# cremebrule/rgb-proprioceptive-pose-estimator

Measured on AMD Instinct MI355X. Metric: images/sec (train step, 224x224 bs256 per GPU), higher is better.
Workload: dtype bf16

## Files before the change

include/rpe_hip.h:

```cpp
#ifndef RPE_HIP_H
#define RPE_HIP_H

#ifdef __cplusplus
extern "C" {
#endif

#define RPE_ABI_VERSION 3

enum { RPE_F32 = 0, RPE_BF16 = 1, RPE_F16 = 2 };
enum {
    RPE_OK = 0,
    RPE_ERR_SHAPE = 1,
    RPE_ERR_DTYPE = 2,
    RPE_ERR_ALIGN = 3,
    RPE_ERR_HIP = 4,
    RPE_ERR_WORKSPACE = 5,
    RPE_ERR_STATE = 6
};

int rpe_abi_version(void);
const char* rpe_build_id(void);
const char* rpe_last_error(void);

typedef struct {
// ... 336 lines not shown
int rpe_resnet50_aux_head_bwd(rpe_resnet50_t* e, const float* dout, long ld_dout, const float* w, const float* depth_feat, const float* raw,
                              const unsigned char* idx, float* dw, float* dbias, float* d_depth_feat, float* workspace, long workspace_floats, void* stream);
int rpe_resnet50_forward(rpe_resnet50_t* e, const float* img_nchw, float* features, long ld_features, int training, void* stream);
int rpe_resnet50_forward_u8(rpe_resnet50_t* e, const unsigned char* frames, int Hs, int Ws, const float* mean3_host, const float* std3_host,
                            float* features, long ld_features, int training, void* stream);
typedef struct {
    int Hr, Wr, top, left, ksx, ksy;
    const int *xb, *xk, *yb, *yk;
    unsigned char* tmp;
} rpe_resize_plan;
int rpe_resnet50_forward_u8_resized(rpe_resnet50_t* e, const unsigned char* frames, int Hs, int Ws, const rpe_resize_plan* rs, const float* mean3_host,
                                    const float* std3_host, float* features, long ld_features, int training, void* stream);
const void* rpe_resnet50_early_feature(const rpe_resnet50_t* e);
void* rpe_resnet50_early_grad(rpe_resnet50_t* e);
int rpe_resnet50_backward(rpe_resnet50_t* e, const float* d_features, long ld_d_features, int use_d_early, void* stream);
enum { RPE_PROF_CONV_FWD = 0, RPE_PROF_CONV_DGRAD = 1, RPE_PROF_CONV_WGRAD = 2, RPE_PROF_BN_FWD = 3, RPE_PROF_BN_BWD = 4,
       RPE_PROF_OTHER = 5, RPE_PROF_NUM = 6 };
int rpe_resnet50_profile(rpe_resnet50_t* e, int enable);
int rpe_resnet50_profile_read(rpe_resnet50_t* e, float* ms, int* launches, double* flops, double* bytes);
long rpe_resnet50_profile_kernels(rpe_resnet50_t* e, char* buf, long buflen);
const char* rpe_last_kernel_name(void);
void rpe_set_walk_direction(int mode);
int rpe_conv2d_wgrad_halo_min_width(int width);
int rpe_resnet50_backward_begin(rpe_resnet50_t* e, const float* d_features, long ld_d_features, void* stream);
int rpe_resnet50_backward_blocks(rpe_resnet50_t* e, int count, int join, void* stream);
int rpe_resnet50_backward_end(rpe_resnet50_t* e, int use_d_early, void* stream);
int rpe_resnet50_backward_frozen(rpe_resnet50_t* e, const float* d_features, long ld_d_features, void* stream);
int rpe_resnet50_set_aux_grad(rpe_resnet50_t* e, const float* aux_dout, long aux_ld, const float* aux_depth_feat, const unsigned char* aux_idx,
                              const float* aux_w);
int rpe_resnet50_tensor(const rpe_resnet50_t* e, const char* name, const void** ptr, long* rows, int* channels);
int rpe_resnet50_set_hook_grad(rpe_resnet50_t* e, int layer, const void* dense_grad);
int rpe_resnet50_set_stem_raw(rpe_resnet50_t* e, int on);

#ifdef __cplusplus
}
#endif
#endif
```

rgb-proprioceptive-pose-estimator_amd/_lib.py:

```python
import ctypes
import os

import torch
from ctypes import POINTER, Structure, c_char_p, c_double, c_float, c_int, c_long, c_void_p

_HERE = os.path.dirname(os.path.abspath(__file__))
LIB_PATH = os.environ.get("RPE_LIB_PATH") or os.path.join(_HERE, "librpe_hip.so")

RPE_F32, RPE_BF16, RPE_F16 = 0, 1, 2
ABI_VERSION = 3
PARAM_STATS_COLS, PARAM_STATS_PART_COLS = 10, 8


class RpeError(RuntimeError):
    """A librpe_hip.so entry point returned a non-zero status."""


class BnBwdEpilogue(Structure):
    _fields_ = [(n, c_void_p) for n in ("y", "a_out", "mean", "invstd", "scale", "shift", "stats_part", "a_mask")]


class ResizePlan(Structure):
    _fields_ = [(n, c_int) for n in ("Hr", "Wr", "top", "left", "ksx", "ksy")] + [(n, c_void_p) for n in ("xb", "xk", "yb", "yk", "tmp")]

# ... 8 lines not shown


class AugmentDesc(Structure):
    _fields_ = ([("seed", ctypes.c_ulonglong)] + [(n, c_int) for n in ("qb_lo", "qb_hi", "qc_lo", "qc_hi", "qs_lo", "qs_hi", "noise_q")]
                + [("erase_thresh", ctypes.c_uint)] + [(n, c_int) for n in ("eh_lo", "eh_hi", "ew_lo", "ew_hi", "fill_mode")]
                + [("fill_rgb", ctypes.c_ubyte * 3), ("group", c_int)])


class SampleDesc(Structure):
    _fields_ = [("seed", ctypes.c_ulonglong)] + [(n, c_int) for n in ("E", "T", "S", "stride", "N", "shuffle")]


class MeasureDesc(Structure):
    _fields_ = [("seed", ctypes.c_ulonglong)] + [(n, c_int) for n in ("S", "N", "num_scales")] + [("sigma", c_double * 8), ("rho", c_double)]


class DropoutDesc(Structure):
    _fields_ = [("seed", ctypes.c_ulonglong), ("thresh", ctypes.c_uint), ("scale", c_float)]


class DepthAugmentDesc(Structure):
    _fields_ = ([("seed", ctypes.c_ulonglong)] + [(n, c_double) for n in ("n0", "n1", "n2", "q", "inv_q", "lo", "hi")] + [("drop_thresh", ctypes.c_uint)]
                + [(n, c_int) for n in ("hole_lo", "hole_hi", "hh_lo", "hh_hi", "hw_lo", "hw_hi")] + [("hole_value", c_float), ("occluder_value", c_float),
                                                                                                       ("group", c_int)])


class OcclusionDesc(Structure):
    _fields_ = [(n, c_int) for n in ("Hs", "Ws", "ph", "pw", "sy", "sx")] + [("fill_rgb", ctypes.c_ubyte * 3)]


class OverlayStyle(Structure):
    _fields_ = [("rgb", ctypes.c_ubyte * 3), ("axis_rgb", ctypes.c_ubyte * 9)] + [(n, c_int) for n in ("alpha_q8", "r_q4", "hw_q4", "trail", "trail_r_q4")]


OVERLAY_INVALID, OVERLAY_NEAR, OVERLAY_CLAMP_Q4, OVERLAY_AXIS_Q4 = -2 ** 31, 2.0 ** -10, 2 ** 17, 2 ** 13
OVERLAY_MAX_SETS, OVERLAY_MAX_TRAIL, OVERLAY_MAX_RADIUS_Q4, OVERLAY_MAX_SIDE = 4, 64, 256, 4096

P, I, L, F, D = c_void_p, c_int, c_long, c_float, c_double
PD = POINTER(ConvDesc)

_SPEC = {
    "rpe_abi_version": (I, []),
    "rpe_last_error": (c_char_p, []),
    "rpe_build_id": (c_char_p, []),
    "rpe_x4_bytes": (L, [I, I, I, I]),
    "rpe_conv_out_hw": (I, [PD, POINTER(c_int), POINTER(c_int)]),
    "rpe_conv_stats_tiles": (L, [L]),
    "rpe_conv2d_fwd": (I, [PD, I, P, P, P, P, P]),
    "rpe_conv2d_fwd_affine": (I, [PD, I, P, P, P, P, P, I, P]),
    "rpe_conv2d_fwd_affine_workspace_bytes": (L, [PD, I]),
    "rpe_conv2d_fwd_affine_ws": (I, [PD, I, P, P, P, P, P, I, P, L, P]),
    "rpe_conv2d_dgrad": (I, [PD, I, P, P, P, P, P]),
    "rpe_conv2d_dgrad_stats_tiles": (L, [PD, I]),
    "rpe_conv2d_fwd_stats_tiles": (L, [PD, I]),
    "rpe_conv2d_dgrad_bn": (I, [PD, I, P, P, P, P, POINTER(BnBwdEpilogue), P]),
    "rpe_conv1x1s2_dgrad_compact": (I, [PD, I, P, P, P, P]),
    "rpe_conv2d_dgrad_sub": (I, [PD, I, P, P, P, P, P]),
    "rpe_conv2d_dgrad_bn_sub": (I, [PD, I, P, P, P, P, POINTER(BnBwdEpilogue), P]),
    "rpe_conv1x1_dgrad_kcat_y_sub": (I, [PD, I, P, P, P, P, P, P, POINTER(BnBwdEpilogue), P]),
    "rpe_bn_backward_reduce": (I, [I, P, P, P, P, P, P, P, P, L, I, P, L, P, P, P]),
    "rpe_bn_backward_from_dz": (I, [I, P, P, P, P, P, P, I, P, P, P, L, I, P, P, P]),
    "rpe_bn_bwd_fold_scratch_bytes": (L, [I, I, I]),
    "rpe_bn_bwd_fold_conv1x1": (I, [I, I, I, P, P, P, P, P, P, P, P, P, L, P]),
    "rpe_conv1x1_dgrad_kcat": (I, [PD, I, P, P, P, P, P, POINTER(BnBwdEpilogue), P]),
    "rpe_bn_bwd_fold_y_conv1x1": (I, [I, I, I, P, P, P, P, P, P, P, P]),
    "rpe_conv1x1_dgrad_kcat_y": (I, [PD, I, P, P, P, P, P, P, POINTER(BnBwdEpilogue), P]),
# ... 105 lines not shown
    "rpe_resnet50_profile": (I, [P, I]),
    "rpe_resnet50_profile_read": (I, [P, POINTER(c_float), POINTER(c_int), POINTER(c_double), POINTER(c_double)]),
    "rpe_resnet50_backward_begin": (I, [P, P, L, P]),
    "rpe_resnet50_backward_blocks": (I, [P, I, I, P]),
    "rpe_resnet50_backward_end": (I, [P, I, P]),
    "rpe_resnet50_backward_frozen": (I, [P, P, L, P]),
    "rpe_resnet50_set_aux_grad": (I, [P, P, L, P, P, P]),
    "rpe_resnet50_profile_kernels": (L, [P, P, L]),
    "rpe_last_kernel_name": (c_char_p, []),
    "rpe_set_walk_direction": (None, [I]),
    "rpe_conv2d_wgrad_halo_min_width": (I, [I]),
    "rpe_resnet50_set_aux_head": (I, [P, P, P, P, P, L, P, P]),
    "rpe_resnet50_aux_head_bwd": (I, [P, P, L, P, P, P, P, P, P, P, P, L, P]),
    "rpe_aux_head_bwd_det_y": (I, [I, P, L, P, P, P, P, P, P, P, P, P, P, I, I, I, P, L, P]),
    "rpe_bn_apply_maxpool3x3s2_aux": (I, [I, P, P, P, P, P, P, I, I, I, P, P, P, P, L, P, P, P]),
    "rpe_resnet50_side_stream_info": (I, [P, POINTER(c_int), POINTER(c_int)]),
    "rpe_resnet50_tensor": (I, [P, c_char_p, POINTER(c_void_p), POINTER(c_long), POINTER(c_int)]),
    "rpe_resnet50_set_hook_grad": (I, [P, I, P]),
    "rpe_resnet50_set_stem_raw": (I, [P, I]),
    "rpe_aux_head_fwd_c": (I, [I, P, I, P, P, P, P, L, P, P, I, I, I, P]),
    "rpe_aux_head_bwd_c": (I, [I, P, L, P, I, P, P, P, P, P, P, P, P, I, I, I, P]),
    "rpe_depth_head_fwd_pools": (I, [P, P, P, P, P, I, I, I, I, P]),
    "rpe_tensor_add": (I, [I, P, P, L, P]),
    "rpe_feature_planes": (I, [I, P, I, I, I, I, P, P, P]),
    "rpe_feature_planes_batch": (I, [I, P, I, I, I, I, P, P, P]),
    "rpe_feature_mosaic": (I, [P, P, I, I, I, I, I, I, P, P]),
    "rpe_occlusion_grid": (L, [POINTER(OcclusionDesc), POINTER(c_int), POINTER(c_int)]),
    "rpe_occlude_grid_u8": (I, [P, P, I, I, POINTER(OcclusionDesc), P]),
    "rpe_pose_displacement": (I, [P, P, L, P, P, P]),
    "rpe_saliency_map": (I, [P, I, POINTER(OcclusionDesc), P, P, P]),
    "rpe_saliency_overlay_u8": (I, [P, P, P, P, I, I, I, I, P, P]),
    "rpe_project_poses": (I, [P, P, P, L, I, I, D, P, P, D, D, I, P, P, P]),
    "rpe_draw_poses_u8": (I, [P, P, L, I, I, P, P, L, I, POINTER(OverlayStyle), I, I, POINTER(ctypes.c_ubyte), I, P]),
}
_NOT_STATUS = {"rpe_abi_version", "rpe_conv2d_wgrad_halo_min_width", "rpe_grad_sumsq_rows", "rpe_param_stats_rows"}

EXPORTS = tuple(_SPEC)


def _load():
    if not os.path.exists(LIB_PATH):
        raise ImportError(
            "librpe_hip.so not found at %s -- build it with `python __graft_entry__.py build` "
            "(hipcc --offload-arch=gfx950); there is no fallback path." % LIB_PATH
        )
    lib = ctypes.CDLL(LIB_PATH)
    for name, (res, args) in _SPEC.items():
        try:
            fn = getattr(lib, name)
        except AttributeError as e:
            raise ImportError("librpe_hip.so does not export %s (stale build?)" % name) from e
        fn.restype = res
        fn.argtypes = args
    if lib.rpe_abi_version() != ABI_VERSION:
        raise ImportError("librpe_hip.so ABI version %d != expected %d" % (lib.rpe_abi_version(), ABI_VERSION))
    return lib


_raw = _load()


class _Checked:

    def __getattr__(self, name):
        fn = getattr(_raw, name)
        res = _SPEC[name][0]
# ... 17 lines not shown
```

rgb-proprioceptive-pose-estimator_amd/headops.py:

```python
import os

import torch

from . import ops
from ._lib import lib

pad4 = ops.pad4


def new_rows(rows, cols, device, zero=True):
    buf = (torch.zeros if zero else torch.empty)((rows, pad4(cols)), dtype=torch.float32, device=device)
    return buf[:, :cols]


def _grad_of(p):
    g = getattr(p, "_rpe_grad", None)
    if g is None:
        raise RuntimeError("parameter has no arena gradient view (model not materialised on the device)")
    return g


class LinearOp:

    def __init__(self, weight, bias, relu=False):
# ... 27 lines not shown
            self.x, self.y = x, out
        return out

    def bwd(self, dy, need_dx=True, accumulate=False):
        n, k = self.weight.shape
        x, y = self.x, self.y
        m = x.shape[0]
        if self.relu:
            if y.stride(0) != pad4(n) or dy.stride(0) != pad4(n):
                raise RuntimeError("LinearOp.bwd: ReLU layers need [M, pad4(N)] row buffers")
            ypad = y.as_strided((m, pad4(n)), (pad4(n), 1), y.storage_offset())
            dypad = dy.as_strided((m, pad4(n)), (pad4(n), 1), dy.storage_offset())
            dy = ops.relu_bwd(ypad, dypad)[:, :n]
        gw = _grad_of(self.weight)
        if k % 4 == 0 and gw.is_contiguous():
            ops.linear_wgrad(dy, x, gw, n=n, k=k, overwrite=not accumulate)
        else:
            tmp = torch.zeros((n, pad4(k)), dtype=torch.float32, device=dy.device)
            ops.linear_wgrad(dy, x, tmp, n=n, k=pad4(k))
            if accumulate:
                gw.add_(tmp[:, :k])
            else:
                ops.copy2d(tmp, gw, cols=k)
        if self.bias is not None:
            ops.colsum(dy, cols=n, out=_grad_of(self.bias), accumulate=accumulate)
        if not need_dx:
            return None
        wt = ops.transpose_f32(self.weight.data, ldo=pad4(n))
        dx = new_rows(m, k, dy.device)
        ops.linear_fwd(dy, wt, None, relu=False, out=dx, n=k, k=pad4(n))
        return dx


class LSTMOp:

    def __init__(self, w_ih, w_hh, b_ih, b_hh):
        self.w_ih, self.w_hh, self.b_ih, self.b_hh = w_ih, w_hh, b_ih, b_hh
        self.in_lin = LinearOp(w_ih, None, relu=False)
        self.hidden = w_hh.shape[1]
        if self.hidden % 4:
            raise ValueError("LSTM hidden size must be a multiple of 4 (16-byte rows)")

    def fwd(self, x, S, N, h0=None, c0=None, save=True):
        H = self.hidden
        dev = x.device
        xg = self.in_lin.fwd(x, save=save)
        gates = torch.empty((S, N, 4 * H), dtype=torch.float32, device=dev)
        hs = torch.empty((S, N, H), dtype=torch.float32, device=dev)
        cs = torch.empty((S, N, H), dtype=torch.float32, device=dev)
        whh = self.w_hh.data
        s = ops._stream()
        for t in range(S):
            h_prev = h0 if t == 0 else hs[t - 1]
            c_prev = c0 if t == 0 else cs[t - 1]
            xg_t = xg[t * N:(t + 1) * N]
            if h_prev is None:
                gates[t].copy_(xg_t)
            else:
                ops.linear_fwd(h_prev, whh, None, addend=xg_t, out=gates[t], n=4 * H, k=H)
            lib.rpe_lstm_cell_fwd(ops._p(gates[t]), ops._p(self.b_ih.data), ops._p(self.b_hh.data), ops._p(c_prev), ops._p(cs[t]), ops._p(hs[t]),
                                  N, H, s)
        if save:
            if h0 is not None:
                h0 = h0.clone()
            if c0 is not None:
                c0 = c0.clone()
# ... 200 lines not shown
```

rgb-proprioceptive-pose-estimator_amd/models/naive.py:

```python
import torch
import torch.nn as nn

from .. import ops
from ..headops import LinearOp, new_rows
from ._core import PoseModelBase, Replicated


class NaiveEndEffectorStateEstimator(PoseModelBase):

    def __init__(self, hidden_dims_pre_measurement, hidden_dims_post_measurement, num_resnet_layers=50, latent_dim=50,
                 feature_extract=True, compute_dtype=None):
        super().__init__()
        self._init_features(num_resnet_layers, latent_dim, feature_extract, True, None, False, wrap=False, register_heads=True,
                            compute_dtype=compute_dtype)
        pre = [latent_dim] + list(hidden_dims_pre_measurement) + [7]
        for i in range(len(pre) - 1):
            setattr(self, "pre_fc{}".format(i), nn.Linear(pre[i], pre[i + 1]))
        self.n_pre_hidden = len(pre) - 1
        post = [latent_dim + 7] + list(hidden_dims_post_measurement) + [7]
        for i in range(len(post) - 1):
            setattr(self, "post_fc{}".format(i), nn.Linear(post[i], post[i + 1]))
        self.n_post_hidden = len(post) - 1
        self._pre_ops = [LinearOp(getattr(self, "pre_fc%d" % i).weight, getattr(self, "pre_fc%d" % i).bias, relu=True)
                         for i in range(self.n_pre_hidden)]
        self._post_ops = [LinearOp(getattr(self, "post_fc%d" % i).weight, getattr(self, "post_fc%d" % i).bias, relu=True)
                          for i in range(self.n_post_hidden)]

    def forward(self, img, depth, self_measurement):
        return self._call(img, depth, self_measurement)

    def _flat_inputs(self, img, depth, x0bar):
        return (img.shape[0],), img, None, x0bar

    def _feature_rows(self, img, depth, save):
        feat = new_rows(img.shape[0], self.latent_dim, img.device)
        self._features_fwd(img, None, feat, save)
        return feat

    def _heads_fwd(self, feat, lead, x0bar, save):
        n, L = feat.shape[0], self.latent_dim
        h = feat
        for op in self._pre_ops:
            h = op.fwd(h, save=save)
        pre = h
        post_in = new_rows(n, L + 7, feat.device)
        ops.copy2d(feat, post_in, cols=L)
        ops.copy2d((pre - x0bar).contiguous(), post_in[:, L:], cols=7)
        h = post_in
        for op in self._post_ops:
            h = op.fwd(h, save=save)
        return pre.contiguous(), h.contiguous()

    def _backward_impl(self, d_outs):
        L = self.latent_dim
        d_pre, d_post = d_outs
        dev = self._pre_ops[0].x.device
        n = self._pre_ops[0].x.shape[0]
        d = self._pad_rows(d_post, 7) if d_post is not None else new_rows(n, 7, dev)
        for op in reversed(self._post_ops):
            d = op.bwd(d)
        d_feat = new_rows(n, L, dev)
        ops.copy2d(d, d_feat, cols=L)
        d_pre_total = d[:, L:L + 7].contiguous()
        if d_pre is not None:
            d_pre_total = d_pre_total + d_pre.reshape(n, 7)
        d = self._pad_rows(d_pre_total, 7)
        for op in reversed(self._pre_ops):
            d = op.bwd(d)
        d_feat.add_(d)
        self._features_bwd(d_feat)

    def reset_initial_state(self, batch_size):
        pass

    @property
    def requires_sequence(self):
        return False


class NaiveObjectStateEstimator(PoseModelBase):

    def __init__(self, object_name, hidden_dims, num_resnet_layers=50, latent_dim=50, feature_extract=True,
                 feature_layer_nums=(9,), use_depth=False, use_pretrained=True, no_proprioception=False, compute_dtype=None):
        super().__init__()
        self.object_name = object_name
        self.use_proprioception = not no_proprioception
        self._init_features(num_resnet_layers, latent_dim, feature_extract, use_pretrained, feature_layer_nums, use_depth, wrap=True,
                            register_heads=True, compute_dtype=compute_dtype)
        print("Latent Dim + Aux Dim = {}".format(latent_dim + self.aux_latent_dim))
        if type(hidden_dims) is int:
            hidden_dims = [hidden_dims]
        input_dim = latent_dim + self.aux_latent_dim + (7 if self.use_proprioception else 0)
        fc_dims = [input_dim] + list(hidden_dims) + [7]
        for i in range(len(fc_dims) - 1):
            setattr(self, "fc{}".format(i), Replicated(nn.Linear(fc_dims[i], fc_dims[i + 1])))
        self.n_fc = len(fc_dims) - 1
        self.input_dim = input_dim
        self._fc_ops = [LinearOp(getattr(self, "fc%d" % i).module.weight, getattr(self, "fc%d" % i).module.bias, relu=True)
                        for i in range(self.n_fc)]

    def forward(self, img, depth, self_measurement):
        return self._call(img, depth, self_measurement)

    def _flat_inputs(self, img, depth, x0bar):
        return (img.shape[0],), img, depth, x0bar

    def _feature_rows(self, img, depth, save):
        rows = new_rows(img.shape[0], self.input_dim, img.device)
        self._features_fwd(img, depth, rows, save)
        return rows

    def _heads_fwd(self, rows, lead, x0bar, save):
        n = rows.shape[0]
        if self.use_proprioception:
            ops.copy2d(x0bar.reshape(n, 7), rows[:, self.latent_dim + self.aux_latent_dim:], cols=7)
        h = rows
        for op in self._fc_ops:
            h = op.fwd(h, save=save)
        return (h.contiguous(),)

    def _backward_impl(self, d_outs):
        d = self._pad_rows(d_outs[0], 7)
        for op in reversed(self._fc_ops):
            d = op.bwd(d)
        self._features_bwd(d)

    def reset_initial_state(self, batch_size):
        pass

    @property
    def requires_sequence(self):
        return False
```

rgb-proprioceptive-pose-estimator_amd/ops.py:

```python
import ctypes
import math
import os

import torch

from ._lib import PARAM_STATS_COLS, PARAM_STATS_PART_COLS, RPE_BF16, RPE_F16, RPE_F32, BnBwdEpilogue, ConvDesc, lib

_DT = {torch.float32: RPE_F32, torch.bfloat16: RPE_BF16, torch.float16: RPE_F16}


def dtype_code(t):
    try:
        return _DT[t if isinstance(t, torch.dtype) else t.dtype]
    except KeyError:
        raise TypeError("unsupported compute dtype %r (fp32, bf16 or fp16)" % (t,))


def _p(t):
    if t is None:
        return None
    if not t.is_cuda:
        raise RuntimeError("librpe_hip ops need device tensors (got a CPU tensor): the HIP path has no CPU fallback")
    return ctypes.c_void_p(t.data_ptr())


def _stream():
    return ctypes.c_void_p(torch.cuda.current_stream().cuda_stream)


def _chk(t, name):
    if not t.is_contiguous():
        raise ValueError("%s must be contiguous" % name)
    return t


def pad4(n):
    return (n + 3) // 4 * 4

# ... 490 lines not shown
        dw.zero_()
    lib.rpe_linear_wgrad(dtype_code(x), _p(dy), dy.stride(0), _p(x), x.stride(0), _p(dw), dw.stride(0), m, n, k, _stream())
    return dw


def transpose_f32(w, ldo=None):
    rows, cols = w.shape
    ldo = pad4(rows) if ldo is None else ldo
    out = torch.empty((cols, ldo), dtype=torch.float32, device=w.device)
    lib.rpe_transpose_f32(_p(w), _p(out), rows, cols, w.stride(0), ldo, _stream())
    return out


def relu_bwd(out, dy):
    dx = torch.empty_like(dy)
    assert out.is_contiguous() and dy.is_contiguous()
    lib.rpe_relu_bwd(_p(out), _p(dy), _p(dx), dy.numel(), _stream())
    return dx


def colsum(x, cols=None, out=None, accumulate=False):
    rows = x.shape[0]
    cols = x.shape[1] if cols is None else cols
    if out is None:
        out = torch.empty(cols, dtype=torch.float32, device=x.device)
    lib.rpe_colsum(_p(x), rows, cols, x.stride(0), _p(out), int(accumulate), _stream())
    return out


def copy2d(src, dst, cols=None):
    cols = src.shape[1] if cols is None else cols
    lib.rpe_copy2d(_p(src), src.stride(0), _p(dst), dst.stride(0), src.shape[0], cols, _stream())
    return dst


def pose_loss(pred, truth, metric, mode, scale, alpha, eps, want_grad=True, valid=None):
    n = pred.numel() // 7
    if valid is not None:
        if not isinstance(valid, torch.Tensor) or valid.dtype not in (torch.uint8, torch.bool) or tuple(valid.shape) != tuple(pred.shape[:-1]):
            raise ValueError("pose_loss: valid must be a uint8 or bool tensor of shape %r; got %s %r" % (
                tuple(pred.shape[:-1]), getattr(valid, "dtype", type(valid)), tuple(getattr(valid, "shape", ()))))
        if valid.device != pred.device or not valid.is_cuda:
            raise ValueError("pose_loss: valid must be on the device of pred (%s); got %s" % (pred.device, valid.device))
        if pred.dtype != torch.float32 or truth.dtype != torch.float32 or truth.device != pred.device:
            raise ValueError("pose_loss: pred and truth must be fp32 on one device")
        _chk(valid, "valid")
        if valid.dtype == torch.bool:
            valid = valid.view(torch.uint8)
    out3 = torch.empty(3, dtype=torch.float32, device=pred.device)
    grad = torch.empty_like(pred) if want_grad else None
    if valid is None:
        lib.rpe_pose_loss(_p(_chk(pred, "pred")), _p(_chk(truth, "truth")), n, metric, mode, scale, alpha, eps, _p(out3), _p(grad), _stream())
    else:
        lib.rpe_pose_loss_masked(_p(_chk(pred, "pred")), _p(_chk(truth, "truth")), _p(valid), n, metric, mode, scale, alpha, eps, _p(out3), _p(grad),
                                 _stream())
    return out3, grad


def pose_errors(pred, truth, eps, want_pose=True):
    if pred.shape != truth.shape or pred.dim() < 1 or pred.shape[-1] != 7:
        raise ValueError("pose_errors: pred and truth must both be (..., 7), got %s and %s" % (tuple(pred.shape), tuple(truth.shape)))
    if pred.dtype != torch.float32 or truth.dtype != torch.float32:
        raise TypeError("pose_errors: pred and truth must be fp32")
    lead = tuple(pred.shape[:-1])
    pos = torch.empty(lead, dtype=torch.float32, device=pred.device)
    ori = torch.empty(lead, dtype=torch.float32, device=pred.device)
# ... 712 lines not shown
```

Measured before the change: 14710.

## Fuse MLP head layer stacks into single-kernel forward and backward tails

Adds HIP kernels that run a chain of small ReLU linear layers in one launch, keeping the per-row activations in LDS between layers, plus a fused backward-data kernel and a batched parameter-gradient kernel covering all tail layers. The pose heads now use an MLPStackOp instead of per-layer LinearOp calls. The aim is to cut per-layer kernel launches and global round trips for the small head MLPs. The costs are new fp32 kernel complexity and large dynamic LDS use. The head is a small share of a ResNet-50 train step.

Result: no change. 14810 (median of 6 runs) (+0.7%).

```diff
diff --git a/include/rpe_hip.h b/include/rpe_hip.h
--- a/include/rpe_hip.h
+++ b/include/rpe_hip.h
@@ -392,6 +392,23 @@
 int rpe_resnet50_set_hook_grad(rpe_resnet50_t* e, int layer, const void* dense_grad);
 int rpe_resnet50_set_stem_raw(rpe_resnet50_t* e, int on);
 
+#define RPE_MLP_MAX_LAYERS 8
+#define RPE_MLP_MAX_WIDTH 1024
+typedef struct {
+    const float* w;
+    const float* b;
+    float* h;
+    float* d;
+    float* dw;
+    float* db;
+    int K, N;
+} rpe_mlp_layer;
+int rpe_mlp_tail_fwd(const rpe_mlp_layer* layers_host, int n_layers, const float* x, int ldx, float* y, int M, int rows_per_group, void* stream);
+int rpe_mlp_tail_bwd_data(const rpe_mlp_layer* layers_host, int n_layers, const float* d_out, int ld_dout, const float* h_in, int ld_hin, float* d_in,
+                          int M, int rows_per_group, void* stream);
+int rpe_mlp_tail_bwd_params(const rpe_mlp_layer* layers_host, int n_layers, const float* h_in, int ld_hin, int M, int accumulate, void* stream);
+int rpe_linear_pack_wide(const float* w, int N, int K, float* w_pad, float* w_t, void* stream);
+
 #ifdef __cplusplus
 }
 #endif
diff --git a/rgb-proprioceptive-pose-estimator_amd/_lib.py b/rgb-proprioceptive-pose-estimator_amd/_lib.py
--- a/rgb-proprioceptive-pose-estimator_amd/_lib.py
+++ b/rgb-proprioceptive-pose-estimator_amd/_lib.py
@@ -64,6 +64,12 @@
 class OverlayStyle(Structure):
     _fields_ = [("rgb", ctypes.c_ubyte * 3), ("axis_rgb", ctypes.c_ubyte * 9)] + [(n, c_int) for n in ("alpha_q8", "r_q4", "hw_q4", "trail", "trail_r_q4")]
 
+
+class MlpLayer(Structure):
+    _fields_ = [(n, c_void_p) for n in ("w", "b", "h", "d", "dw", "db")] + [("K", c_int), ("N", c_int)]
+
+
+MLP_MAX_LAYERS, MLP_MAX_WIDTH = 8, 1024
 
 OVERLAY_INVALID, OVERLAY_NEAR, OVERLAY_CLAMP_Q4, OVERLAY_AXIS_Q4 = -2 ** 31, 2.0 ** -10, 2 ** 17, 2 ** 13
 OVERLAY_MAX_SETS, OVERLAY_MAX_TRAIL, OVERLAY_MAX_RADIUS_Q4, OVERLAY_MAX_SIDE = 4, 64, 256, 4096
@@ -235,6 +241,10 @@
     "rpe_saliency_overlay_u8": (I, [P, P, P, P, I, I, I, I, P, P]),
     "rpe_project_poses": (I, [P, P, P, L, I, I, D, P, P, D, D, I, P, P, P]),
     "rpe_draw_poses_u8": (I, [P, P, L, I, I, P, P, L, I, POINTER(OverlayStyle), I, I, POINTER(ctypes.c_ubyte), I, P]),
+    "rpe_mlp_tail_fwd": (I, [POINTER(MlpLayer), I, P, I, P, I, I, P]),
+    "rpe_mlp_tail_bwd_data": (I, [POINTER(MlpLayer), I, P, I, P, I, P, I, I, P]),
+    "rpe_mlp_tail_bwd_params": (I, [POINTER(MlpLayer), I, P, I, I, I, P]),
+    "rpe_linear_pack_wide": (I, [P, I, I, P, P, P]),
 }
 _NOT_STATUS = {"rpe_abi_version", "rpe_conv2d_wgrad_halo_min_width", "rpe_grad_sumsq_rows", "rpe_param_stats_rows"}
 
diff --git a/rgb-proprioceptive-pose-estimator_amd/csrc/mlp_stack.hip b/rgb-proprioceptive-pose-estimator_amd/csrc/mlp_stack.hip
--- /dev/null
+++ b/rgb-proprioceptive-pose-estimator_amd/csrc/mlp_stack.hip
@@ -0,0 +1,429 @@
+#include <string.h>
+
+#include "common.h"
+
+using namespace rpe;
+
+namespace {
+
+constexpr int kFwdThreads = 512;
+constexpr int kBwdThreads = 512;
+constexpr int kMaxLds = 160 * 1024;
+
+struct TailArgs {
+    rpe_mlp_layer l[RPE_MLP_MAX_LAYERS];
+    int n_layers;
+    const float* x;
+    int ldx;
+    float* y;
+    const float* d_out;
+    int ld_dout;
+    int M, LD;
+    int accumulate;
+    int tile_start[RPE_MLP_MAX_LAYERS + 1];
+};
+
+__device__ __forceinline__ int pad4i(int n) { return (n + 3) & ~3; }
+
+template <int N, int OFF> __device__ __forceinline__ void halve_step(float (&v)[32], int lane) {
+    const bool up = (lane & OFF) != 0;
+#pragma unroll
+    for (int i = 0; i < N; ++i) {
+        const float send = up ? v[i] : v[i + N];
+        const float keep = up ? v[i + N] : v[i];
+        v[i] = keep + __shfl_xor(send, OFF, 64);
+    }
+}
+__device__ __forceinline__ float reduce_values(float (&v)[32], int lane) {
+    halve_step<16, 32>(v, lane);
+    halve_step<8, 16>(v, lane);
+    halve_step<4, 8>(v, lane);
+    halve_step<2, 4>(v, lane);
+    halve_step<1, 2>(v, lane);
+    return v[0] + __shfl_xor(v[0], 1, 64);
+}
+
+template <int R> __global__ __launch_bounds__(kFwdThreads) void mlp_tail_fwd_kernel(TailArgs a) {
+    constexpr int CB = 32 / R, V = 32;
+    extern __shared__ f32x4 lds4[];
+    float* cur = (float*)lds4;
+    float* nxt = cur + R * a.LD;
+    const int tid = threadIdx.x, lane = tid & 63, wave = tid >> 6;
+    const int LD = a.LD, M = a.M;
+    const long row0 = (long)blockIdx.x * R;
+    {
+        const int K0 = a.l[0].K;
+        for (int i = tid; i < R * K0; i += kFwdThreads) {
+            const int r = i / K0, c = i - r * K0;
+            const long m = row0 + r;
+            cur[r * LD + c] = m < M ? a.x[m * a.ldx + c] : 0.f;
+        }
+    }
+    __syncthreads();
+    for (int li = 0; li < a.n_layers; ++li) {
+        const rpe_mlp_layer L = a.l[li];
+        const int K = L.K, N = L.N;
+        const bool vec = !(K & 3) && !(((uintptr_t)L.w) & 15);
+        const int my = lane >> 1, myc = my / R, myr = my - myc * R;
+        for (int n0 = wave * CB; n0 < N; n0 += (kFwdThreads / 64) * CB) {
+            float acc[V];
+#pragma unroll
+            for (int i = 0; i < V; ++i) acc[i] = 0.f;
+            const float bias = n0 + myc < N ? L.b[n0 + myc] : 0.f;
+            const float* wr[CB];
+#pragma unroll
+            for (int c = 0; c < CB; ++c) wr[c] = L.w + (long)(n0 + c < N ? n0 + c : N - 1) * K;
+            if (vec) {
+#pragma unroll 4
+                for (int k4 = lane; k4 < (K >> 2); k4 += 64) {
+                    f32x4 w[CB];
+#pragma unroll
+                    for (int c = 0; c < CB; ++c) w[c] = ((const f32x4*)wr[c])[k4];
+#pragma unroll
+                    for (int r = 0; r < R; ++r) {
+                        const f32x4 h = ((const f32x4*)(cur + r * LD))[k4];
+#pragma unroll
+                        for (int c = 0; c < CB; ++c)
+                            acc[c * R + r] = fmaf(h.w, w[c].w, fmaf(h.z, w[c].z, fmaf(h.y, w[c].y, fmaf(h.x, w[c].x, acc[c * R + r]))));
+                    }
+                }
+            } else {
+#pragma unroll 1
+                for (int k = lane; k < K; k += 64) {
+                    float w[CB];
+#pragma unroll
+                    for (int c = 0; c < CB; ++c) w[c] = wr[c][k];
+#pragma unroll
+                    for (int r = 0; r < R; ++r) {
+                        const float h = cur[r * LD + k];
+#pragma unroll
+                        for (int c = 0; c < CB; ++c) acc[c * R + r] = fmaf(h, w[c], acc[c * R + r]);
+                    }
+                }
+            }
+            const float v = reduce_values(acc, lane);
+            if (!(lane & 1) && n0 + myc < N) nxt[myr * LD + n0 + myc] = fmaxf(v + bias, 0.f);
+        }
+        __syncthreads();
+        const int Np = pad4i(N);
+        if (L.h) {
+            for (int i = tid; i < R * Np; i += kFwdThreads) {
+                const int r = i / Np, c = i - r * Np;
+                const long m = row0 + r;
+                if (m < M) L.h[m * Np + c] = c < N ? nxt[r * LD + c] : 0.f;
+            }
+        }
+        if (li == a.n_layers - 1) {
+            for (int i = tid; i < R * N; i += kFwdThreads) {
+                const int r = i / N, c = i - r * N;
+                const long m = row0 + r;
+                if (m < M) a.y[m * N + c] = nxt[r * LD + c];
+            }
+        }
+        float* t = cur; cur = nxt; nxt = t;
+    }
+}
+
+template <int RT, bool VEC> __device__ __forceinline__ void dgrad_units(const float* __restrict__ W, int K, int N, const float* dl, float* dn, int LD,
+                                                                        int r0, int ut, int gt) {
+    const int U = VEC ? (K >> 2) : K;
+    const int Np = pad4i(N);
+    for (int u = ut; u < U; u += gt) {
+        if constexpr (VEC) {
+            f32x4 acc[RT];
+#pragma unroll
+            for (int r = 0; r < RT; ++r) acc[r] = f32x4{0.f, 0.f, 0.f, 0.f};
+            const f32x4 z = {0.f, 0.f, 0.f, 0.f};
+#pragma unroll 2
+            for (int n = 0; n < Np; n += 4) {
+                const f32x4* w4 = (const f32x4*)(W + (long)n * K) + u;
+                const int kq = K >> 2;
+                const f32x4 w0 = w4[0];
+                const f32x4 w1 = n + 1 < N ? w4[kq] : z;
+                const f32x4 w2 = n + 2 < N ? w4[2 * kq] : z;
+                const f32x4 w3 = n + 3 < N ? w4[3 * kq] : z;
+#pragma unroll
+                for (int r = 0; r < RT; ++r) {
+                    const f32x4 d = *(const f32x4*)(dl + (r0 + r) * LD + n);
+                    acc[r] = acc[r] + d.x * w0;
+                    acc[r] = acc[r] + d.y * w1;
+                    acc[r] = acc[r] + d.z * w2;
+                    acc[r] = acc[r] + d.w * w3;
+                }
+            }
+#pragma unroll
+            for (int r = 0; r < RT; ++r) *(f32x4*)(dn + (r0 + r) * LD + 4 * u) = acc[r];
+        } else {
+            float acc[RT];
+#pragma unroll
+            for (int r = 0; r < RT; ++r) acc[r] = 0.f;
+            for (int n = 0; n < N; ++n) {
+                const float w = W[(long)n * K + u];
+#pragma unroll
+                for (int r = 0; r < RT; ++r) acc[r] = fmaf(dl[(r0 + r) * LD + n], w, acc[r]);
+            }
+#pragma unroll
+            for (int r = 0; r < RT; ++r) dn[(r0 + r) * LD + u] = acc[r];
+        }
+    }
+}
+
+template <bool VEC> __device__ __forceinline__ void dgrad_layer(const float* W, int K, int N, const float* dl, float* dn, int LD, int R, int tid) {
+    const int U = VEC ? (K >> 2) : K;
+    const int Uw = (U + 63) & ~63;
+    int RG = 1;
+    while (RG * 2 <= R && RG * 2 * Uw <= kBwdThreads) RG *= 2;
+    const int gt = kBwdThreads / RG, rg = tid / gt, ut = tid - rg * gt;
+    const int RT = R / RG, r0 = rg * RT;
+    switch (RT) {
+    case 1: dgrad_units<1, VEC>(W, K, N, dl, dn, LD, r0, ut, gt); break;
+    case 2: dgrad_units<2, VEC>(W, K, N, dl, dn, LD, r0, ut, gt); break;
+    case 4: dgrad_units<4, VEC>(W, K, N, dl, dn, LD, r0, ut, gt); break;
+    case 8: dgrad_units<8, VEC>(W, K, N, dl, dn, LD, r0, ut, gt); break;
+    default: dgrad_units<16, VEC>(W, K, N, dl, dn, LD, r0, ut, gt); break;
+    }
+}
+
+__device__ __forceinline__ void mask_store(float* buf, int LD, const float* src, int ld_src, const float* h, int ldh, float* out, int C, long row0, int M,
+                                           int R, int tid) {
+    const int Cp = pad4i(C);
+    for (int i = tid; i < R * Cp; i += kBwdThreads) {
+        const int r = i / Cp, c = i - r * Cp;
+        const long m = row0 + r;
+        float v = 0.f;
+        if (m < M && c < C) {
+            v = src ? src[m * ld_src + c] : buf[r * LD + c];
+            v = h[m * ldh + c] > 0.f ? v : 0.f;
+        }
+        buf[r * LD + c] = v;
+        if (m < M) out[m * Cp + c] = v;
+    }
+}
+
+__global__ __launch_bounds__(kBwdThreads) void mlp_tail_bwd_data_kernel(TailArgs a, int R) {
+    extern __shared__ f32x4 lds4[];
+    float* cur = (float*)lds4;
+    float* nxt = cur + R * a.LD;
+    const int tid = threadIdx.x, LD = a.LD, M = a.M;
+    const long row0 = (long)blockIdx.x * R;
+    {
+        const rpe_mlp_layer& L = a.l[a.n_layers - 1];
+        mask_store(cur, LD, a.d_out, a.ld_dout, L.h, pad4i(L.N), L.d, L.N, row0, M, R, tid);
+    }
+    __syncthreads();
+    for (int li = a.n_layers - 1; li >= 0; --li) {
+        const rpe_mlp_layer L = a.l[li];
+        const int K = L.K, N = L.N;
+        if (!(K & 3) && !(((uintptr_t)L.w) & 15)) dgrad_layer<true>(L.w, K, N, cur, nxt, LD, R, tid);
+        else dgrad_layer<false>(L.w, K, N, cur, nxt, LD, R, tid);
+        __syncthreads();
+        if (li > 0) mask_store(nxt, LD, nullptr, 0, a.l[li - 1].h, pad4i(K), a.l[li - 1].d, K, row0, M, R, tid);
+        else mask_store(nxt, LD, nullptr, 0, a.x, a.ldx, a.y, K, row0, M, R, tid);
+        __syncthreads();
+        float* t = cur; cur = nxt; nxt = t;
+    }
+}
+
+constexpr int kPN = 16, kPK = 64, kPChunk = 256;
+
+__global__ __launch_bounds__(256) void mlp_tail_bwd_params_kernel(TailArgs a) {
+    __shared__ f32x4 dsh[kPChunk][kPN / 4];
+    __shared__ float red[4][kPN][kPK];
+    __shared__ float redb[4][kPN];
+    const int tid = threadIdx.x, lane = tid & 63, wave = tid >> 6;
+    int li = 0;
+    while (li + 1 < a.n_layers && (int)blockIdx.x >= a.tile_start[li + 1]) ++li;
+    const rpe_mlp_layer L = a.l[li];
+    const int K = L.K, N = L.N, Np = pad4i(N), M = a.M;
+    const int t = blockIdx.x - a.tile_start[li], tiles_k = (K + kPK - 1) / kPK;
+    const int n0 = (t / tiles_k) * kPN, k0 = (t % tiles_k) * kPK;
+    const float* H = li > 0 ? a.l[li - 1].h : a.x;
+    const int ldh = li > 0 ? pad4i(K) : a.ldx;
+    const int k = k0 + lane;
+    const bool kok = k < K, want_db = k0 == 0 && tid < 4 * kPN;
+    float acc[kPN];
+#pragma unroll
+    for (int j = 0; j < kPN; ++j) acc[j] = 0.f;
+    float bsum = 0.f;
+    for (int mc = 0; mc < M; mc += kPChunk) {
+        const int cnt = M - mc < kPChunk ? M - mc : kPChunk;
+        if (tid < cnt) {
+            const float* dr = L.d + (long)(mc + tid) * Np + n0;
+#pragma unroll
+            for (int q = 0; q < kPN / 4; ++q) dsh[tid][q] = n0 + 4 * q < Np ? *(const f32x4*)(dr + 4 * q) : f32x4{0.f, 0.f, 0.f, 0.f};
+        }
+        __syncthreads();
+        const int i1 = (wave + 1) * 64 < cnt ? (wave + 1) * 64 : cnt;
+        if (kok) {
+            const float* hp = H + (long)mc * ldh + k;
+#pragma unroll 8
+            for (int i = wave * 64; i < i1; ++i) {
+                const float h = hp[(long)i * ldh];
+#pragma unroll
+                for (int q = 0; q < kPN / 4; ++q) {
+                    const f32x4 d = dsh[i][q];
+                    acc[4 * q] = fmaf(d.x, h, acc[4 * q]);
+                    acc[4 * q + 1] = fmaf(d.y, h, acc[4 * q + 1]);
+                    acc[4 * q + 2] = fmaf(d.z, h, acc[4 * q + 2]);
+                    acc[4 * q + 3] = fmaf(d.w, h, acc[4 * q + 3]);
+                }
+            }
+        }
+        if (want_db) {
+            const int j = tid & (kPN - 1), part = tid / kPN;
+            const int e = (part + 1) * 64 < cnt ? (part + 1) * 64 : cnt;
+            for (int i = part * 64; i < e; ++i) bsum += ((const float*)&dsh[i][0])[j];
+        }
+        __syncthreads();
+    }
+#pragma unroll
+    for (int j = 0; j < kPN; ++j) red[wave][j][lane] = acc[j];
+    if (want_db) redb[tid / kPN][tid & (kPN - 1)] = bsum;
+    __syncthreads();
+    if (kok) {
+#pragma unroll
+        for (int jj = 0; jj < kPN / 4; ++jj) {
+            const int j = wave * (kPN / 4) + jj, n = n0 + j;
+            if (n < N) {
+                const float v = ((red[0][j][lane] + red[1][j][lane]) + red[2][j][lane]) + red[3][j][lane];
+                float* p = L.dw + (long)n * K + k;
+                *p = a.accumulate ? *p + v : v;
+            }
+        }
+    }
+    if (k0 == 0 && tid < kPN && n0 + tid < N) {
+        const float v = ((redb[0][tid] + redb[1][tid]) + redb[2][tid]) + redb[3][tid];
+        float* p = L.db + n0 + tid;
+        *p = a.accumulate ? *p + v : v;
+    }
+}
+
+__global__ __launch_bounds__(256) void linear_pack_wide_kernel(const float* __restrict__ w, int N, int K, float* __restrict__ wpad, float* __restrict__ wt) {
+    __shared__ float tile[32][33];
+    const int Kp = pad4i(K), Np = pad4i(N);
+    const int bx = blockIdx.x * 32, by = blockIdx.y * 32;
+    const int tx = threadIdx.x & 31, ty = threadIdx.x >> 5;
+    for (int i = ty; i < 32; i += 8) {
+        const int n = by + i, k = bx + tx;
+        const float v = (n < N && k < K) ? w[(long)n * K + k] : 0.f;
+        tile[i][tx] = v;
+        if (wpad && n < N && k < Kp) wpad[(long)n * Kp + k] = v;
+    }
+    __syncthreads();
+    if (!wt) return;
+    for (int i = ty; i < 32; i += 8) {
+        const int k = bx + i, n = by + tx;
+        if (k < Kp && n < Np) wt[(long)k * Np + n] = tile[tx][i];
+    }
+}
+
+int check_layers(const rpe_mlp_layer* l, int n, int M, int R, bool bwd, const char* who, int* LD) {
+    static thread_local char msg[160];
+    if (!l || n < 1 || n > RPE_MLP_MAX_LAYERS || M < 1 || (R != 8 && R != 16)) {
+        snprintf(msg, sizeof(msg), "%s: 1..%d layers, M >= 1, rows_per_group 8 or 16", who, RPE_MLP_MAX_LAYERS);
+        return rpe_set_error(RPE_ERR_SHAPE, msg);
+    }
+    int widest = l[0].K;
+    for (int i = 0; i < n; ++i) {
+        if (l[i].K < 1 || l[i].N < 1 || l[i].K > RPE_MLP_MAX_WIDTH || l[i].N > RPE_MLP_MAX_WIDTH || (i > 0 && l[i].K != l[i - 1].N)) {
+            snprintf(msg, sizeof(msg), "%s: layer widths must lie in 1..%d and chain (K of a layer = N of the one before)", who, RPE_MLP_MAX_WIDTH);
+            return rpe_set_error(RPE_ERR_SHAPE, msg);
+        }
+        if (!l[i].w || !l[i].b || (bwd && (!l[i].h || !l[i].d))) {
+            snprintf(msg, sizeof(msg), "%s: layer %d lacks a pointer", who, i);
+            return rpe_set_error(RPE_ERR_SHAPE, msg);
+        }
+        if ((((uintptr_t)l[i].h) & 15) || (((uintptr_t)l[i].d) & 15)) {
+            snprintf(msg, sizeof(msg), "%s: row buffers must be 16-byte aligned", who);
+            return rpe_set_error(RPE_ERR_ALIGN, msg);
+        }
+        if (l[i].N > widest) widest = l[i].N;
+    }
+    *LD = (widest + 3) & ~3;
+    return 0;
+}
+
+template <typename Kern> int raise_lds(Kern kern, bool& done) {
+    if (done) return 0;
+    hipError_t e = hipFuncSetAttribute((const void*)kern, hipFuncAttributeMaxDynamicSharedMemorySize, kMaxLds);
+    if (e != hipSuccess) return rpe_set_error_hip(e, __FILE__, __LINE__);
+    done = true;
+    return 0;
+}
+
+}
+
+extern "C" {
+
+int rpe_mlp_tail_fwd(const rpe_mlp_layer* layers_host, int n_layers, const float* x, int ldx, float* y, int M, int rows_per_group, void* stream) {
+    TailArgs a;
+    memset(&a, 0, sizeof(a));
+    if (int e = check_layers(layers_host, n_layers, M, rows_per_group, false, "mlp_tail_fwd", &a.LD)) return e;
+    if (!x || !y || ldx < layers_host[0].K) return rpe_set_error(RPE_ERR_SHAPE, "mlp_tail_fwd: x [M][ldx >= K], y [M][N_last]");
+    for (int i = 0; i < n_layers; ++i) a.l[i] = layers_host[i];
+    a.n_layers = n_layers; a.x = x; a.ldx = ldx; a.y = y; a.M = M;
+    const int R = rows_per_group;
+    const size_t lds = (size_t)2 * R * a.LD * sizeof(float);
+    const dim3 grid((unsigned)((M + R - 1) / R));
+    note_kernel("mlp_tail_fwd_kernel");
+    static bool raised8 = false, raised16 = false;
+    if (R == 8) {
+        if (int e = raise_lds(mlp_tail_fwd_kernel<8>, raised8)) return e;
+        hipLaunchKernelGGL((mlp_tail_fwd_kernel<8>), grid, dim3(kFwdThreads), lds, (hipStream_t)stream, a);
+    } else {
+        if (int e = raise_lds(mlp_tail_fwd_kernel<16>, raised16)) return e;
+        hipLaunchKernelGGL((mlp_tail_fwd_kernel<16>), grid, dim3(kFwdThreads), lds, (hipStream_t)stream, a);
+    }
+    RPE_CHECK_LAUNCH();
+    return 0;
+}
+
+int rpe_mlp_tail_bwd_data(const rpe_mlp_layer* layers_host, int n_layers, const float* d_out, int ld_dout, const float* h_in, int ld_hin, float* d_in,
+                          int M, int rows_per_group, void* stream) {
+    TailArgs a;
+    memset(&a, 0, sizeof(a));
+    if (int e = check_layers(layers_host, n_layers, M, rows_per_group, true, "mlp_tail_bwd_data", &a.LD)) return e;
+    if (!d_out || !h_in || !d_in || ld_dout < layers_host[n_layers - 1].N || ld_hin < layers_host[0].K || (((uintptr_t)d_in) & 15))
+        return rpe_set_error(RPE_ERR_SHAPE, "mlp_tail_bwd_data: d_out [M][ld >= N_last], h_in [M][ld >= K_first], d_in [M][pad4(K_first)] 16-byte aligned");
+    for (int i = 0; i < n_layers; ++i) a.l[i] = layers_host[i];
+    a.n_layers = n_layers; a.x = h_in; a.ldx = ld_hin; a.y = d_in; a.d_out = d_out; a.ld_dout = ld_dout; a.M = M;
+    const int R = rows_per_group;
+    const size_t lds = (size_t)2 * R * a.LD * sizeof(float);
+    note_kernel("mlp_tail_bwd_data_kernel");
+    static bool raised = false;
+    if (int e = raise_lds(mlp_tail_bwd_data_kernel, raised)) return e;
+    hipLaunchKernelGGL(mlp_tail_bwd_data_kernel, dim3((unsigned)((M + R - 1) / R)), dim3(kBwdThreads), lds, (hipStream_t)stream, a, R);
+    RPE_CHECK_LAUNCH();
+    return 0;
+}
+
+int rpe_mlp_tail_bwd_params(const rpe_mlp_layer* layers_host, int n_layers, const float* h_in, int ld_hin, int M, int accumulate, void* stream) {
+    TailArgs a;
+    memset(&a, 0, sizeof(a));
+    if (int e = check_layers(layers_host, n_layers, M, 8, true, "mlp_tail_bwd_params", &a.LD)) return e;
+    if (!h_in || ld_hin < layers_host[0].K) return rpe_set_error(RPE_ERR_SHAPE, "mlp_tail_bwd_params: h_in [M][ld >= K_first]");
+    int tiles = 0;
+    for (int i = 0; i < n_layers; ++i) {
+        if (!layers_host[i].dw || !layers_host[i].db) return rpe_set_error(RPE_ERR_SHAPE, "mlp_tail_bwd_params: a layer lacks dw / db");
+        a.l[i] = layers_host[i];
+        a.tile_start[i] = tiles;
+        tiles += ((layers_host[i].N + kPN - 1) / kPN) * ((layers_host[i].K + kPK - 1) / kPK);
+    }
+    a.tile_start[n_layers] = tiles;
+    a.n_layers = n_layers; a.x = h_in; a.ldx = ld_hin; a.M = M; a.accumulate = accumulate;
+    note_kernel("mlp_tail_bwd_params_kernel");
+    hipLaunchKernelGGL(mlp_tail_bwd_params_kernel, dim3((unsigned)tiles), dim3(256), 0, (hipStream_t)stream, a);
+    RPE_CHECK_LAUNCH();
+    return 0;
+}
+
+int rpe_linear_pack_wide(const float* w, int N, int K, float* w_pad, float* w_t, void* stream) {
+    if (!w || N < 1 || K < 1 || (!w_pad && !w_t)) return rpe_set_error(RPE_ERR_SHAPE, "linear_pack_wide: w [N][K] and at least one image");
+    const int Kp = (K + 3) & ~3, Np = (N + 3) & ~3;
+    note_kernel("linear_pack_wide_kernel");
+    hipLaunchKernelGGL(linear_pack_wide_kernel, dim3((Kp + 31) / 32, (Np + 31) / 32), dim3(256), 0, (hipStream_t)stream, w, N, K, w_pad, w_t);
+    RPE_CHECK_LAUNCH();
+    return 0;
+}
+
+}
diff --git a/rgb-proprioceptive-pose-estimator_amd/headops.py b/rgb-proprioceptive-pose-estimator_amd/headops.py
--- a/rgb-proprioceptive-pose-estimator_amd/headops.py
+++ b/rgb-proprioceptive-pose-estimator_amd/headops.py
@@ -83,6 +83,89 @@
         return dx
 
 
+class MLPStackOp:
+
+    fused = True
+
+    def __init__(self, layers):
+        self.ops = [LinearOp(w, b, relu=True) for w, b in layers]
+        self._wpad = None
+        self._saved = self.kept = None
+
+    def takes_fused(self, rows):
+        if not self.fused or len(self.ops) < 2 or len(self.ops) - 1 > ops.MLP_MAX_LAYERS or rows <= ops.LINEAR_ROWS_MAX:
+            return False
+        for i, op in enumerate(self.ops):
+            if op.bias is None or not op.weight.data.is_contiguous() or not op.bias.data.is_contiguous():
+                return False
+            if i > 0 and max(op.weight.shape) > ops.MLP_MAX_WIDTH:
+                return False
+        return True
+
+    def fwd(self, x, save=True):
+        m, dev = x.shape[0], x.device
+        if not self.takes_fused(m):
+            h = x
+            for op in self.ops:
+                h = op.fwd(h, save=save)
+            if save:
+                self._saved = None
+            return h.contiguous()
+        op0 = self.ops[0]
+        n0, k0 = op0.weight.shape
+        w0 = op0.weight.data
+        wt = torch.empty((pad4(k0), pad4(n0)), dtype=torch.float32, device=dev) if save else None
+        wp = None
+        if k0 % 4:
+            if self._wpad is None or self._wpad.device != dev:
+                self._wpad = torch.empty((n0, pad4(k0)), dtype=torch.float32, device=dev)
+            wp = self._wpad
+        if wp is not None or wt is not None:
+            ops.linear_pack_wide(w0, wp, wt)
+        y0 = new_rows(m, n0, dev, zero=n0 % 4 != 0)
+        ops.linear_fwd(x, w0 if wp is None else wp, op0.bias.data, relu=True, out=y0, n=n0, k=pad4(k0))
+        hs = [torch.empty((m, pad4(op.weight.shape[0])), dtype=torch.float32, device=dev) if save else None for op in self.ops[1:]]
+        y = torch.empty((m, self.ops[-1].weight.shape[0]), dtype=torch.float32, device=dev)
+        ops.mlp_tail_fwd(ops.mlp_layers([dict(w=op.weight.data, b=op.bias.data, h=h) for op, h in zip(self.ops[1:], hs)]), y0, y)
+        if save:
+            self._saved = (x, y0, wt, hs)
+        return y
+
+    def bwd(self, d_out, need_dx=True, accumulate=False):
+        n_last = self.ops[-1].weight.shape[0]
+        d_out = d_out.reshape(-1, n_last).float()
+        m, dev = d_out.shape[0], d_out.device
+        if self._saved is None:
+            d = new_rows(m, n_last, dev)
+            ops.copy2d(d_out.contiguous(), d, cols=n_last)
+            for i in reversed(range(len(self.ops))):
+                d = self.ops[i].bwd(d, need_dx=need_dx or i > 0, accumulate=accumulate)
+            return d
+        x, y0, wt, hs = self._saved
+        if d_out.stride(1) != 1:
+            d_out = d_out.contiguous()
+        op0 = self.ops[0]
+        n0, k0 = op0.weight.shape
+        entries = [dict(w=op.weight.data, b=op.bias.data, h=h, d=torch.empty_like(h), dw=_grad_of(op.weight), db=_grad_of(op.bias))
+                   for op, h in zip(self.ops[1:], hs)]
+        layers = ops.mlp_layers(entries)
+        dy0 = torch.empty((m, pad4(n0)), dtype=torch.float32, device=dev)
+        ops.mlp_tail_bwd_data(layers, d_out, y0, dy0)
+        ops.mlp_tail_bwd_params(layers, y0, m, accumulate=accumulate)
+        self.kept = (dy0, [e["d"] for e in entries], d_out)
+        dy0 = dy0[:, :n0]
+        gw = _grad_of(op0.weight)
+        if not gw.is_contiguous():
+            raise RuntimeError("MLPStackOp.bwd: the first layer's gradient view must be contiguous")
+        ops.linear_wgrad(dy0, x, gw, n=n0, k=k0, overwrite=not accumulate)
+        ops.colsum(dy0, cols=n0, out=_grad_of(op0.bias), accumulate=accumulate)
+        if not need_dx:
+            return None
+        dx = torch.empty((m, pad4(k0)), dtype=torch.float32, device=dev)
+        ops.linear_fwd(dy0, wt, None, relu=False, out=dx, n=pad4(k0), k=pad4(n0))
+        return dx[:, :k0]
+
+
 class LSTMOp:
 
     def __init__(self, w_ih, w_hh, b_ih, b_hh):
diff --git a/rgb-proprioceptive-pose-estimator_amd/models/naive.py b/rgb-proprioceptive-pose-estimator_amd/models/naive.py
--- a/rgb-proprioceptive-pose-estimator_amd/models/naive.py
+++ b/rgb-proprioceptive-pose-estimator_amd/models/naive.py
@@ -2,7 +2,7 @@
 import torch.nn as nn
 
 from .. import ops
-from ..headops import LinearOp, new_rows
+from ..headops import MLPStackOp, new_rows
 from ._core import PoseModelBase, Replicated
 
 
@@ -21,10 +21,8 @@
         for i in range(len(post) - 1):
             setattr(self, "post_fc{}".format(i), nn.Linear(post[i], post[i + 1]))
         self.n_post_hidden = len(post) - 1
-        self._pre_ops = [LinearOp(getattr(self, "pre_fc%d" % i).weight, getattr(self, "pre_fc%d" % i).bias, relu=True)
-                         for i in range(self.n_pre_hidden)]
-        self._post_ops = [LinearOp(getattr(self, "post_fc%d" % i).weight, getattr(self, "post_fc%d" % i).bias, relu=True)
-                          for i in range(self.n_post_hidden)]
+        self._pre_stack = MLPStackOp([(getattr(self, "pre_fc%d" % i).weight, getattr(self, "pre_fc%d" % i).bias) for i in range(self.n_pre_hidden)])
+        self._post_stack = MLPStackOp([(getattr(self, "post_fc%d" % i).weight, getattr(self, "post_fc%d" % i).bias) for i in range(self.n_post_hidden)])
 
     def forward(self, img, depth, self_measurement):
         return self._call(img, depth, self_measurement)
@@ -39,35 +37,24 @@
 
     def _heads_fwd(self, feat, lead, x0bar, save):
         n, L = feat.shape[0], self.latent_dim
-        h = feat
-        for op in self._pre_ops:
-            h = op.fwd(h, save=save)
-        pre = h
+        pre = self._pre_stack.fwd(feat, save=save)
         post_in = new_rows(n, L + 7, feat.device)
         ops.copy2d(feat, post_in, cols=L)
         ops.copy2d((pre - x0bar).contiguous(), post_in[:, L:], cols=7)
-        h = post_in
-        for op in self._post_ops:
-            h = op.fwd(h, save=save)
-        return pre.contiguous(), h.contiguous()
+        return pre, self._post_stack.fwd(post_in, save=save)
 
     def _backward_impl(self, d_outs):
         L = self.latent_dim
         d_pre, d_post = d_outs
-        dev = self._pre_ops[0].x.device
-        n = self._pre_ops[0].x.shape[0]
-        d = self._pad_rows(d_post, 7) if d_post is not None else new_rows(n, 7, dev)
-        for op in reversed(self._post_ops):
-            d = op.bwd(d)
+        n = (d_post if d_post is not None else d_pre).numel() // 7
+        dev = self.pre_fc0.weight.device
+        d = self._post_stack.bwd(d_post if d_post is not None else torch.zeros((n, 7), dtype=torch.float32, device=dev))
         d_feat = new_rows(n, L, dev)
         ops.copy2d(d, d_feat, cols=L)
         d_pre_total = d[:, L:L + 7].contiguous()
         if d_pre is not None:
             d_pre_total = d_pre_total + d_pre.reshape(n, 7)
-        d = self._pad_rows(d_pre_total, 7)
-        for op in reversed(self._pre_ops):
-            d = op.bwd(d)
-        d_feat.add_(d)
+        d_feat.add_(self._pre_stack.bwd(d_pre_total))
         self._features_bwd(d_feat)
 
     def reset_initial_state(self, batch_size):
@@ -96,8 +83,7 @@
             setattr(self, "fc{}".format(i), Replicated(nn.Linear(fc_dims[i], fc_dims[i + 1])))
         self.n_fc = len(fc_dims) - 1
         self.input_dim = input_dim
-        self._fc_ops = [LinearOp(getattr(self, "fc%d" % i).module.weight, getattr(self, "fc%d" % i).module.bias, relu=True)
-                        for i in range(self.n_fc)]
+        self._fc_stack = MLPStackOp([(getattr(self, "fc%d" % i).module.weight, getattr(self, "fc%d" % i).module.bias) for i in range(self.n_fc)])
 
     def forward(self, img, depth, self_measurement):
         return self._call(img, depth, self_measurement)
@@ -114,16 +100,10 @@
         n = rows.shape[0]
         if self.use_proprioception:
             ops.copy2d(x0bar.reshape(n, 7), rows[:, self.latent_dim + self.aux_latent_dim:], cols=7)
-        h = rows
-        for op in self._fc_ops:
-            h = op.fwd(h, save=save)
-        return (h.contiguous(),)
+        return (self._fc_stack.fwd(rows, save=save),)
 
     def _backward_impl(self, d_outs):
-        d = self._pad_rows(d_outs[0], 7)
-        for op in reversed(self._fc_ops):
-            d = op.bwd(d)
-        self._features_bwd(d)
+        self._features_bwd(self._fc_stack.bwd(d_outs[0]))
 
     def reset_initial_state(self, batch_size):
         pass
diff --git a/rgb-proprioceptive-pose-estimator_amd/ops.py b/rgb-proprioceptive-pose-estimator_amd/ops.py
--- a/rgb-proprioceptive-pose-estimator_amd/ops.py
+++ b/rgb-proprioceptive-pose-estimator_amd/ops.py
@@ -4,6 +4,7 @@
 
 import torch
 
+from . import _lib
 from ._lib import PARAM_STATS_COLS, PARAM_STATS_PART_COLS, RPE_BF16, RPE_F16, RPE_F32, BnBwdEpilogue, ConvDesc, lib
 
 _DT = {torch.float32: RPE_F32, torch.bfloat16: RPE_BF16, torch.float16: RPE_F16}
@@ -560,6 +561,50 @@
     cols = src.shape[1] if cols is None else cols
     lib.rpe_copy2d(_p(src), src.stride(0), _p(dst), dst.stride(0), src.shape[0], cols, _stream())
     return dst
+
+
+MLP_MAX_LAYERS, MLP_MAX_WIDTH = _lib.MLP_MAX_LAYERS, _lib.MLP_MAX_WIDTH
+MLP_ROWS_PER_GROUP = 8
+
+
+def mlp_layers(entries):
+    arr = (_lib.MlpLayer * len(entries))()
+    for a, e in zip(arr, entries):
+        w = _chk(e["w"], "mlp layer weight")
+        a.N, a.K = w.shape
+        a.w, a.b = w.data_ptr(), _chk(e["b"], "mlp layer bias").data_ptr()
+        for name in ("h", "d", "dw", "db"):
+            t = e.get(name)
+            if t is not None:
+                if name in ("h", "d") and (t.stride(0) != pad4(a.N) or t.stride(1) != 1):
+                    raise ValueError("mlp_layers: %s must be rows of an [M, pad4(N)] buffer" % name)
+                if name in ("dw", "db"):
+                    _chk(t, "mlp layer " + name)
+                setattr(a, name, t.data_ptr())
+    return arr
+
+
+def mlp_tail_fwd(layers, x, y, rows_per_group=None):
+    lib.rpe_mlp_tail_fwd(layers, len(layers), _p(x), x.stride(0), _p(_chk(y, "y")), x.shape[0], rows_per_group or MLP_ROWS_PER_GROUP, _stream())
+    return y
+
+
+def mlp_tail_bwd_data(layers, d_out, h_in, d_in, rows_per_group=None):
+    lib.rpe_mlp_tail_bwd_data(layers, len(layers), _p(d_out), d_out.stride(0), _p(h_in), h_in.stride(0), _p(d_in), d_out.shape[0],
+                              rows_per_group or MLP_ROWS_PER_GROUP, _stream())
+    return d_in
+
+
+def mlp_tail_bwd_params(layers, h_in, rows, accumulate=False):
+    lib.rpe_mlp_tail_bwd_params(layers, len(layers), _p(h_in), h_in.stride(0), rows, int(accumulate), _stream())
+
+
+def linear_pack_wide(w, w_pad=None, w_t=None):
+    n, k = _chk(w, "w").shape
+    for t, shape in ((w_pad, (n, pad4(k))), (w_t, (pad4(k), pad4(n)))):
+        if t is not None and (tuple(t.shape) != shape or not t.is_contiguous()):
+            raise ValueError("linear_pack_wide: an image must be contiguous %r" % (shape,))
+    lib.rpe_linear_pack_wide(_p(w), n, k, _p(w_pad), _p(w_t), _stream())
 
 
 def pose_loss(pred, truth, metric, mode, scale, alpha, eps, want_grad=True, valid=None):
```
